# kuailehaha/liuzhou

Hardware: AMD Instinct MI355X
Metric: self-play positions/sec (fixed sims/move) (higher is better)
Workload: dtype f16

## Files before the change

include/liuzhou_hip.h:

```cpp
#ifndef LIUZHOU_HIP_H
#define LIUZHOU_HIP_H

#include <stdint.h>

#ifdef __cplusplus
extern "C" {
#endif

#if defined(_WIN32)
#define LZ_API
#else
#define LZ_API __attribute__((visibility("default")))
#endif

typedef enum LzStatus {
    LZ_OK = 0,
    LZ_ERR_ARG = -1,
    LZ_ERR_UNSUPPORTED = -2,
    LZ_ERR_LAUNCH = -3,
    LZ_ERR_ALIGN = -4,
    LZ_ERR_ILLEGAL = -5
} LzStatus;


// ... 110 lines not shown
                          float* arena_state, uint8_t* arena_legal, float* arena_policy, float* arena_value,
                          float* arena_soft, int8_t* arena_sign, void* stream);

LZ_API int lz_wave_step_finish(const LzStateSoA* states, int64_t num_slots, int64_t* plies, uint8_t* done,
                               const int32_t* chosen_action_codes, const uint8_t* terminal_mask,
                               const uint8_t* chosen_valid_mask, int64_t max_game_plies, float soft_value_k,
                               float* value_targets, float* soft_value_targets, const int8_t* player_signs,
                               const int64_t* step_index_matrix, int64_t* step_counts, int64_t max_steps,
                               int64_t* outcome, int64_t* delta_hist, int64_t* lengths, const int64_t* slot_game,
                               int64_t* finished, uint8_t* reseated, int reseat, void* stream);

LZ_API int lz_wave_reseat(const LzStateSoA* states, int64_t num_slots, uint8_t* done, int64_t* plies,
                          int64_t* step_counts, int64_t* budget, int64_t* next_game, int64_t* slot_game,
                          uint8_t* reseated, int logged_only, void* stream);

LZ_API int lz_wave_log_finished(const uint8_t* done, int64_t* step_counts, int64_t num_slots, int64_t max_steps,
                                int64_t action_dim, const float* arena_state, const uint8_t* arena_legal,
                                const float* arena_policy, const float* arena_value, const float* arena_soft,
                                float* log_state_rows, uint8_t* log_legal, float* log_policy, float* log_value,
                                float* log_soft, int64_t log_capacity, int64_t* log_state, int64_t* log_base,
                                void* stream);


#define LZ_NET_MAX_LAYERS 96
typedef struct LzNetDesc {
    int32_t channels;
    int32_t blocks;
    int32_t num_layers;
    int32_t max_blocks;
    const void* wfrag;
    const float* fparams;
    int64_t wfrag_bytes;
    int64_t fparams_bytes;
    int32_t layer_offsets[LZ_NET_MAX_LAYERS];
    int32_t head_frag_offsets[4];
    int32_t off_stem_bias, off_block0 , off_trunk_a, off_trunk_b,
            off_head_bias, off_p_gwT, off_p_a2, off_p_b2, off_p_out, off_v_w1T, off_v_b1, off_v_w2T, off_v_b2;
    int32_t flags;
    const float* wfrag_f32;
    int64_t wfrag_f32_bytes;
    const void* wfrag_lo;
    int64_t wfrag_lo_bytes;
} LzNetDesc;

LZ_API int lz_net_forward_f16(const LzNetDesc* net, const float* planes, int64_t batch,
                              float* log_p1, float* log_p2, float* log_pmc,
                              float* value_logits, float* value, void* stream);
LZ_API int lz_net_forward_packed_f16(const LzNetDesc* net, const void* packed_states, int64_t batch,
                                     float* log_p1, float* log_p2, float* log_pmc,
                                     float* value_logits, float* value, void* stream);
LZ_API int lz_net_forward_packed_counted_f16(const LzNetDesc* net, const void* packed_states, int64_t capacity,
                                             const int64_t* count, float* log_p1, float* log_p2, float* log_pmc,
                                             float* value_logits, float* value, void* stream);
LZ_API int lz_net_configure(void);
LZ_API int64_t lz_net_desc_bytes(void);
LZ_API int lz_prof_enable(int on);
LZ_API int lz_prof_net_summary(double* total_ms, int64_t* launches, int64_t* evals);
LZ_API int lz_prof_net_busy(double* busy_ms);
LZ_API int lz_prof_aux_summary(int kind, double* total_ms, int64_t* launches, int64_t* units);


typedef struct LzTreeDesc {
    int64_t num_games;
    int32_t node_cap, edge_chunk , path_cap, chunk_cap;
    double  exploration_weight;
    const void* root_state;
    void*    nodes;
    void*    edges;
    int32_t* n_nodes;
    int32_t* n_edges;
    int32_t* root_visits;
    double*  root_w;
    float*   root_init_value;
    int32_t* path;
    int32_t* path_len;
    int32_t* leaf_kind;
    void*    leaf_state;
    float*   leaf_value;
    uint8_t* root_terminal;
    const uint8_t* active;
    int32_t* leaf_edge;
    int32_t* leaf_parent;
    int32_t* trace_kind;
    void*    trace_leaf;
    float*   trace_heads;
    float*   trace_priors;
    float*   trace_value;
    int64_t  trace_cap;
    int32_t* eval_count;
    int32_t* chunk_list;
    int32_t* n_chunks;
    int32_t* free_chunks;
    int32_t* pool_top;
    int32_t* pool_stats;
    int64_t  pool_chunks;
    void*    live_state;
    int32_t* live_row;
    int64_t* live_count;
    int64_t  live_count_cap;
    int32_t* pos_index;
    float*   node_value;
    int32_t* leaf_src;
    int32_t* share_count;
    int64_t  pos_slots;
} LzTreeDesc;
LZ_API int64_t lz_tree_desc_bytes(void);
// ... 105 lines not shown
```

liuzhou_amd/csrc/lz_engine.hip:

```cpp
#include <hip/hip_runtime.h>
#include <hip/amd_detail/amd_hip_unsafe_atomics.h>
#include <math.h>
#include <stdint.h>

#include <mutex>

#include "lz_rng.h"
#include "lz_tree_dev.h"

namespace {

__global__ __launch_bounds__(kBlock) void pack_states_kernel(LzStateSoA s, int64_t B, Packed* __restrict__ out) {
    const int64_t i = (int64_t)blockIdx.x * kBlock + threadIdx.x;
    if (i >= B) return;
    State st;
    st.black = cells_equal(s.board + i * 36, 1);
    st.white = cells_equal(s.board + i * 36, -1);
    st.mb = cells_nonzero(s.marks_black + i * 36);
    st.mw = cells_nonzero(s.marks_white + i * 36);
    st.phase = (int)s.phase[i]; st.player = (int)s.current_player[i];
    st.pm_req = (int)s.pending_marks_required[i]; st.pm_rem = (int)s.pending_marks_remaining[i];
    st.pc_req = (int)s.pending_captures_required[i]; st.pc_rem = (int)s.pending_captures_remaining[i];
    st.forced = (int)s.forced_removals_done[i]; st.move_count = (int)s.move_count[i];
    st.msc = (int)s.moves_since_capture[i];
// ... 1132 lines not shown

int lz_prof_aux_begin(int kind, void* stream);
int lz_prof_aux_end(int kind, void* stream, int64_t units);

int lz_tree_advance(const LzTreeDesc* d, const int32_t* played_action, const uint8_t* reset, int64_t next_sims,
                    int32_t* dropped, int32_t* pruned, void* stream) {
    if (!tree_ok(d) || next_sims < 0) return LZ_ERR_ARG;
    if (d->num_games == 0) return LZ_OK;
    const int words = (d->node_cap + kWave - 1) / kWave;
    if (words > kMarkWordsBig) return LZ_ERR_UNSUPPORTED;
    const int64_t rn = next_sims + 1;
    if (rn > d->node_cap) return LZ_ERR_ARG;
    if ((int64_t)d->chunk_cap * (d->edge_chunk - (kMaxChildren - 1)) < (int64_t)d->node_cap * kMaxChildren) return LZ_ERR_ARG;
    const bool big = words > kMarkWordsMax;
    const int wpb = big ? 1 : kWavesPerBlock;
    const size_t lds = (size_t)wpb * (words * (sizeof(uint64_t) + sizeof(int)) + 3 * kWave * sizeof(int));
    if (big) {
        static std::mutex mu;
        static bool configured[64] = {};
        int dev = 0;
        if (hipGetDevice(&dev) != hipSuccess || dev < 0 || dev >= 64) return LZ_ERR_LAUNCH;
        std::lock_guard<std::mutex> lk(mu);
        if (!configured[dev]) {
            const size_t most = (size_t)kMarkWordsBig * (sizeof(uint64_t) + sizeof(int)) + 3 * kWave * sizeof(int);
            if (hipFuncSetAttribute(reinterpret_cast<const void*>(tree_advance_kernel<1>),
                                    hipFuncAttributeMaxDynamicSharedMemorySize, (int)most) != hipSuccess) {
                (void)hipGetLastError();
                return LZ_ERR_LAUNCH;
            }
            configured[dev] = true;
        }
    }
    (void)lz_prof_aux_begin(1, stream);
    if (big)
        hipLaunchKernelGGL(tree_advance_kernel<1>, dim3((unsigned)d->num_games), dim3(kWave), lds, as_stream(stream), make_tree(d),
                           played_action, reset, (int)rn, words, dropped, pruned, g_advance_ticks);
    else
        hipLaunchKernelGGL(tree_advance_kernel<kWavesPerBlock>, dim3(gw(d->num_games)), dim3(kBlock), lds, as_stream(stream),
                           make_tree(d), played_action, reset, (int)rn, words, dropped, pruned, g_advance_ticks);
    (void)lz_prof_aux_end(1, stream, d->num_games);
    return st();
}

static int tree_search_impl(const LzTreeDesc* d, const LzNetDesc* net, int64_t sims, float* planes, float* lp1,
                            float* lp2, float* lpmc, float* values, const float* noise, int64_t noise_stride,
                            float epsilon, bool continue_trees, void* stream) {
    if (!tree_ok(d) || !net || sims < 0 || !lp1 || !lp2 || !lpmc || !values) return LZ_ERR_ARG;
    const int64_t B = d->num_games;
    if (B == 0) return LZ_OK;
    int rc = continue_trees ? LZ_OK : lz_tree_begin(d, stream);
    if (rc) return rc;
    (void)planes;
    const Tree t = split_step(B) ? no_share(make_tree(d)) : make_tree(d);
    if (t.live_count != nullptr) {
        if (d->live_count_cap < sims + 2) return LZ_ERR_ARG;
        hipLaunchKernelGGL(tree_live_scan_kernel, dim3(1), dim3(kScanBlock), 0, as_stream(stream), t, t.live_count);
        for (int64_t s = 0; s <= sims; ++s) {
            rc = lz_net_forward_packed_counted_f16(net, d->live_state, B, d->live_count + s, lp1, lp2, lpmc, nullptr, values,
                                                   stream);
            if (rc) return rc;
            if (s == sims) {
                if (s == 0)
                    hipLaunchKernelGGL((tree_expand_kernel<true, true>), dim3(gw(t.B)), dim3(kBlock), 0, as_stream(stream), t,
                                       lp1, lp2, lpmc, (const float*)nullptr, values, noise, (int)noise_stride, epsilon, (int)s);
                else
                    hipLaunchKernelGGL((tree_expand_kernel<false, true>), dim3(gw(t.B)), dim3(kBlock), 0, as_stream(stream), t,
                                       lp1, lp2, lpmc, (const float*)nullptr, values, (const float*)nullptr, 0, 0.f, (int)s);
            } else if (s == 0) {
                hipLaunchKernelGGL((tree_expand_select_kernel<true, true>), dim3(gw(t.B)), dim3(kBlock), 0, as_stream(stream),
                                   t, lp1, lp2, lpmc, values, noise, (int)noise_stride, epsilon, (int)s);
            } else {
                (void)lz_prof_aux_begin(0, stream);
                if (split_step(t.B))
                    hipLaunchKernelGGL((tree_expand_select_split_kernel<true>), dim3(gw2(t.B)), dim3(kBlock), 0,
                                       as_stream(stream), t, lp1, lp2, lpmc, values, (int)s);
                else
                    hipLaunchKernelGGL((tree_expand_select_kernel<false, true>), dim3(gw(t.B)), dim3(kBlock), 0, as_stream(stream),
                                       t, lp1, lp2, lpmc, values, nullptr, 0, 0.f, (int)s);
                (void)lz_prof_aux_end(0, stream, B);
            }
            if (s < sims)
                hipLaunchKernelGGL(tree_live_scan_kernel, dim3(1), dim3(kScanBlock), 0, as_stream(stream), t,
                                   t.live_count + (s + 1));
        }
        return st();
    }
    for (int64_t s = 0; s <= sims; ++s) {
        rc = lz_net_forward_packed_f16(net, d->leaf_state, B, lp1, lp2, lpmc, nullptr, values, stream);
        if (rc) return rc;
        if (s == sims) {
            if (s == 0)
                hipLaunchKernelGGL(tree_expand_kernel<true>, dim3(gw(t.B)), dim3(kBlock), 0, as_stream(stream), t, lp1, lp2,
                                   lpmc, (const float*)nullptr, values, noise, (int)noise_stride, epsilon, (int)s);
            else
                hipLaunchKernelGGL(tree_expand_kernel<false>, dim3(gw(t.B)), dim3(kBlock), 0, as_stream(stream), t, lp1, lp2,
                                   lpmc, (const float*)nullptr, values, (const float*)nullptr, 0, 0.f, (int)s);
        } else if (s == 0) {
            hipLaunchKernelGGL(tree_expand_select_kernel<true>, dim3(gw(t.B)), dim3(kBlock), 0, as_stream(stream), t, lp1,
                               lp2, lpmc, values, noise, (int)noise_stride, epsilon, (int)s);
        } else {
            (void)lz_prof_aux_begin(0, stream);
            if (split_step(t.B))
                hipLaunchKernelGGL((tree_expand_select_split_kernel<false>), dim3(gw2(t.B)), dim3(kBlock), 0, as_stream(stream),
                                   t, lp1, lp2, lpmc, values, (int)s);
            else
                hipLaunchKernelGGL(tree_expand_select_kernel<false>, dim3(gw(t.B)), dim3(kBlock), 0, as_stream(stream), t, lp1,
                                   lp2, lpmc, values, nullptr, 0, 0.f, (int)s);
            (void)lz_prof_aux_end(0, stream, B);
        }
    }
    return st();
}

#ifdef LZ_EXP_TREE_STAMPS
LZ_API int lz_exp_tree_stamps(unsigned long long* out32, int reset) {
    if (out32 && hipMemcpyFromSymbol(out32, HIP_SYMBOL(g_tree_stamps), 32 * sizeof(unsigned long long)) != hipSuccess) return LZ_ERR_LAUNCH;
    if (reset) {
        unsigned long long z[32] = {};
        if (hipMemcpyToSymbol(HIP_SYMBOL(g_tree_stamps), z, sizeof(z)) != hipSuccess) return LZ_ERR_LAUNCH;
    }
    return LZ_OK;
}
#endif

int64_t lz_tree_desc_bytes(void) { return (int64_t)sizeof(LzTreeDesc); }

int lz_root_prepare(const void* root_states, int64_t B, const float* lp1, const float* lp2, const float* lpmc,
                    const float* noise, float epsilon, int64_t* legal_index_mat, float* priors_mat,
                    int32_t* action_code_mat, uint8_t* valid_mask, int32_t* counts, uint8_t* terminal_mask,
                    float* leaf_mat, void* child_states, int32_t* child_ref, uint64_t* n_children,
                    int64_t child_capacity, int32_t* overflow, void* stream) {
    if (B < 0) return LZ_ERR_ARG;
    if (B == 0) return LZ_OK;
    if (!root_states || !lp1 || !lp2 || !lpmc || !legal_index_mat || !priors_mat || !action_code_mat || !valid_mask ||
        !counts || !terminal_mask || !leaf_mat || !child_states || !child_ref || !n_children || child_capacity < 0)
        return LZ_ERR_ARG;
    if (reinterpret_cast<uintptr_t>(action_code_mat) & 15) return LZ_ERR_ALIGN;
    hipLaunchKernelGGL(zero_u64_kernel, dim3(1), dim3(64), 0, as_stream(stream),
                       reinterpret_cast<unsigned long long*>(n_children));
    hipLaunchKernelGGL(root_prepare_kernel, dim3(gw(B)), dim3(kBlock), 0, as_stream(stream),
                       reinterpret_cast<const Packed*>(root_states), B, lp1, lp2, lpmc, noise, epsilon, legal_index_mat,
// ... 122 lines not shown
```

liuzhou_amd/csrc/lz_net.hip:

```cpp
#include <hip/hip_runtime.h>
#include <algorithm>
#include <utility>
#include <vector>
#include <math.h>
#include <stdint.h>
#include <stdlib.h>

#include "../../include/liuzhou_hip.h"
#include "lz_net_dev.h"

namespace {

template <int C, int S, int W>
__global__ __launch_bounds__(W * 64, (C == 128 && W == 4) ? 1 : 2) void net_forward_kernel(NetParams P, const float* __restrict__ planes,
                                                            const uint64_t* __restrict__ packed,
                                                            int64_t N, float* __restrict__ lp1,
                                                            float* __restrict__ lp2, float* __restrict__ lpm,
                                                            float* __restrict__ vlogits, float* __restrict__ value) {
    if (P.n_dev != nullptr) { const long long nd = *P.n_dev; N = nd < N ? nd : N; }
    extern __shared__ __attribute__((aligned(16))) unsigned char lds[];
    NetCtx<C, S, W> ctx;
#ifdef LZ_EXP_HEAD_STAMPS
    ctx.t_entry = __builtin_readcyclecounter();
#endif
    net_setup<C, S, W>(P, lds, ctx);
#ifdef LZ_EXP_HEAD_STAMPS
    asm volatile("s_waitcnt vmcnt(0) lgkmcnt(0)" ::: "memory");
    ctx.t_setup = __builtin_readcyclecounter();
#endif
    const uint64_t dbg_t0 = P.debug_stop == 99 ? __builtin_readcyclecounter() : 0;
    const uint64_t dbg_w0 = P.debug_stop == 99 ? wall_clock64() : 0;
    const int64_t n_pass = (N + S - 1) / S;
    for (int64_t pass = blockIdx.x; pass < n_pass; pass += gridDim.x) {
        const int64_t n0 = pass * S;
        const int nvalid = (int)((N - n0) < S ? (N - n0) : S);
        net_pass<C, S, W>(P, lds, ctx, planes, packed, n0, nvalid, lp1, lp2, lpm, vlogits, value);
    }
    if (P.debug_stop == 99 && blockIdx.x == 7 && threadIdx.x == 0) {
        const uint64_t dt = __builtin_readcyclecounter() - dbg_t0, dw = wall_clock64() - dbg_w0;
        value[0] = (float)dt; value[1] = (float)dw;
    }
}

template <int C, int S, int W>
int launch_net(const NetParams& P, const float* planes, const uint64_t* packed, int64_t N, float* lp1, float* lp2,
               float* lpm, float* vlogits, float* value, int max_blocks, hipStream_t st) {
    using K = Cfg<C, S, W>;
    auto kern = net_forward_kernel<C, S, W>;
    const int64_t n_pass = (N + S - 1) / S;
    int grid = (int)(n_pass < max_blocks ? n_pass : max_blocks);
    if (grid < 1) grid = 1;
    hipLaunchKernelGGL(kern, dim3(grid), dim3(K::THREADS), K::LDS_BYTES, st, P, planes, packed, N, lp1, lp2, lpm, vlogits, value);
    return hipGetLastError() == hipSuccess ? LZ_OK : LZ_ERR_LAUNCH;
}

template <int C, int S, int W>
int configure_net() {
    return hipFuncSetAttribute(reinterpret_cast<const void*>(net_forward_kernel<C, S, W>),
                               hipFuncAttributeMaxDynamicSharedMemorySize, Cfg<C, S, W>::LDS_BYTES) == hipSuccess
               ? LZ_OK : LZ_ERR_LAUNCH;
}

}

namespace {
struct NetProf {
    bool on = false;
    int used = 0;
    static constexpr int kMax = 8192;
    hipEvent_t ev[2 * kMax];
    bool created = false;
    double flops = 0.0;
    int64_t evals = 0;
} g_prof;
}

extern "C" void lz_prof_aux_reset(void);

extern "C" {

int lz_prof_enable(int on) {
    if (on && !g_prof.created) {
        for (int i = 0; i < 2 * NetProf::kMax; ++i)
            if (hipEventCreate(&g_prof.ev[i]) != hipSuccess) return LZ_ERR_LAUNCH;
        g_prof.created = true;
    }
    g_prof.on = on != 0;
    g_prof.used = 0;
    g_prof.evals = 0;
    lz_prof_aux_reset();
    return LZ_OK;
}

int lz_prof_net_summary(double* total_ms, int64_t* launches, int64_t* evals) {
    double t = 0.0;
    for (int i = 0; i < g_prof.used; ++i) {
        float ms = 0.f;
        if (hipEventElapsedTime(&ms, g_prof.ev[2 * i], g_prof.ev[2 * i + 1]) != hipSuccess) return LZ_ERR_LAUNCH;
        t += ms;
    }
    if (total_ms) *total_ms = t;
    if (launches) *launches = g_prof.used;
    if (evals) *evals = g_prof.evals;
    return LZ_OK;
}

int lz_prof_net_busy(double* busy_ms) {
    if (!busy_ms) return LZ_ERR_ARG;
    *busy_ms = 0.0;
    const int n = g_prof.used;
// ... 80 lines not shown
    return a != LZ_OK ? a : (b != LZ_OK ? b : (c != LZ_OK ? c : e));
}

int lz_net_forward_f32_dispatch(const LzNetDesc* d, const float* planes, const uint64_t* packed, int64_t N, float* lp1,
                                float* lp2, float* lpmc, float* value_logits, float* value, const int64_t* n_dev,
                                void* stream);

static int net_forward_impl(const LzNetDesc* d, const float* planes, const uint64_t* packed, int64_t N, float* lp1,
                            float* lp2, float* lpmc, float* value_logits, float* value, void* stream,
                            const int64_t* n_dev = nullptr) {
    if (!d || N < 0) return LZ_ERR_ARG;
    if (N == 0) return LZ_OK;
    if (!d->wfrag || !d->fparams || (!planes && !packed)) return LZ_ERR_ARG;
    const bool heads = lp1 && lp2 && lpmc;
    if (!heads && (lp1 || lp2 || lpmc || !value)) return LZ_ERR_ARG;
    if (d->blocks < 0 || d->blocks > (LZ_NET_MAX_LAYERS - 2) / 2 || d->num_layers != 2 + 2 * d->blocks) return LZ_ERR_ARG;
    if ((reinterpret_cast<uintptr_t>(d->wfrag) & 15) || (reinterpret_cast<uintptr_t>(d->fparams) & 15)) return LZ_ERR_ALIGN;
    if (d->flags & (4 | 8))
        return lz_net_forward_f32_dispatch(d, planes, packed, N, lp1, lp2, lpmc, value_logits, value, n_dev, stream);
    NetParams P = make_net_params(d);
#ifdef LZ_EXP_SAME_LAYER
    for (int i = 3; i < 1 + 2 * d->blocks; ++i) P.layer_off[i] = d->layer_offsets[1 + ((i - 1) & 1)];
#endif
    P.n_dev = reinterpret_cast<const long long*>(n_dev);
    P.debug_stop = getenv("LZ_NET_DEBUG_STOP") ? atoi(getenv("LZ_NET_DEBUG_STOP")) : 0;
    const bool half_wg = d->channels == 64 && (d->flags & 1);
    const int max_blocks = d->max_blocks > 0 ? d->max_blocks : (half_wg ? 512 : 256);
    hipStream_t st = reinterpret_cast<hipStream_t>(stream);
    if (d->channels != 64 && d->channels != 128) return LZ_ERR_UNSUPPORTED;
    const bool prof = g_prof.on && g_prof.used < NetProf::kMax;
    if (prof) (void)hipEventRecord(g_prof.ev[2 * g_prof.used], st);
    const bool wide = d->channels == 128 && (d->flags & 2);
    const int rc = d->channels == 64
                       ? (half_wg
                              ? launch_net<64, 8, 4>(P, planes, packed, N, lp1, lp2, lpmc, value_logits, value, max_blocks, st)
                              : launch_net<64, 16, 8>(P, planes, packed, N, lp1, lp2, lpmc, value_logits, value, max_blocks, st))
                       : (wide ? launch_net<128, 8, 4>(P, planes, packed, N, lp1, lp2, lpmc, value_logits, value, max_blocks, st)
                               : launch_net<128, 8, 8>(P, planes, packed, N, lp1, lp2, lpmc, value_logits, value, max_blocks, st));
    if (prof) { (void)hipEventRecord(g_prof.ev[2 * g_prof.used + 1], st); g_prof.used += 1; g_prof.evals += N; }
    return rc;
}

int lz_net_forward_f16(const LzNetDesc* d, const float* planes, int64_t N, float* lp1, float* lp2, float* lpmc,
                       float* value_logits, float* value, void* stream) {
    return net_forward_impl(d, planes, nullptr, N, lp1, lp2, lpmc, value_logits, value, stream);
}

int lz_net_forward_packed_f16(const LzNetDesc* d, const void* packed_states, int64_t N, float* lp1, float* lp2,
                              float* lpmc, float* value_logits, float* value, void* stream) {
    return net_forward_impl(d, nullptr, reinterpret_cast<const uint64_t*>(packed_states), N, lp1, lp2, lpmc,
                            value_logits, value, stream);
}

int lz_net_forward_packed_counted_f16(const LzNetDesc* d, const void* packed_states, int64_t capacity,
                                      const int64_t* count, float* lp1, float* lp2, float* lpmc, float* value_logits,
                                      float* value, void* stream) {
    if (!count) return LZ_ERR_ARG;
    return net_forward_impl(d, nullptr, reinterpret_cast<const uint64_t*>(packed_states), capacity, lp1, lp2, lpmc,
                            value_logits, value, stream, count);
}

}
```

liuzhou_amd/csrc/lz_net_dev.h:

```cpp
#pragma once
#include <hip/hip_runtime.h>
#include <math.h>
#include <stdint.h>

#include "../../include/liuzhou_hip.h"
#include "lz_wave.h"

namespace {


typedef _Float16 h8 __attribute__((ext_vector_type(8)));
typedef _Float16 h4 __attribute__((ext_vector_type(4)));
typedef float f4 __attribute__((ext_vector_type(4)));
typedef unsigned int u4 __attribute__((ext_vector_type(4)));

struct Rsrc { __amdgpu_buffer_rsrc_t w, f; };
__device__ __forceinline__ __amdgpu_buffer_rsrc_t make_rsrc(const void* p, int bytes) {
    return __builtin_amdgcn_make_buffer_rsrc(const_cast<void*>(p), 0, bytes, 0x00020000);
}
__device__ __forceinline__ h8 load_wfrag(__amdgpu_buffer_rsrc_t r, int lane_off, int byte_off) {
    return __builtin_bit_cast(h8, __builtin_amdgcn_raw_buffer_load_b128(r, lane_off, byte_off, 0));
}
__device__ __forceinline__ f4 load_f4(__amdgpu_buffer_rsrc_t r, int lane_float_off, int float_off) {
    return __builtin_bit_cast(f4, __builtin_amdgcn_raw_buffer_load_b128(r, lane_float_off * 4, float_off * 4, 0));
// ... 364 lines not shown
__device__ __forceinline__ void fc_load(__amdgpu_buffer_rsrc_t rw, int half_off, int ct, int lane, h8 (&a)[KBN]) {
    const int wbyte = __builtin_amdgcn_readfirstlane(half_off * 2 + ct * 1024);
#pragma unroll
    for (int kb = 0; kb < KBN; ++kb) a[kb] = load_wfrag(rw, lane * 16, wbyte + kb * CTN * 1024);
}
template <int KBN>
__device__ __forceinline__ f4 fc_mma(const h8 (&a)[KBN], const unsigned char* rows, int row_stride, int lane) {
    f4 d = (f4){0.f, 0.f, 0.f, 0.f};
    const unsigned char* bp = rows + (lane & 15) * row_stride + (lane >> 4) * 16;
#pragma unroll
    for (int kb = 0; kb < KBN; ++kb)
        d = __builtin_amdgcn_mfma_f32_16x16x32_f16(a[kb], *reinterpret_cast<const h8*>(bp + kb * 64), d, 0, 0, 0);
    return d;
}
template <int CTN, int KBN>
__device__ __forceinline__ f4 fc_tile(__amdgpu_buffer_rsrc_t rw, int half_off, int ct,
                                      const unsigned char* rows, int row_stride, int lane) {
    h8 a[KBN];
    fc_load<CTN, KBN>(rw, half_off, ct, lane, a);
    return fc_mma<KBN>(a, rows, row_stride, lane);
}

template <int C, int S, int NW>
__device__ __forceinline__ void store_head(const AccT<NW>& acc, unsigned char* lds, const int (&base)[9], int map_tile0,
                                           __amdgpu_buffer_rsrc_t rf, int bias_off, int lane) {
    const int sub = (lane >> 4) * 4;
    const int delta = store_delta<C, S>(map_tile0 * 16, lane);
    f4 b[NW];
#pragma unroll
    for (int j = 0; j < NW; ++j) b[j] = load_f4(rf, sub, bias_off + (map_tile0 + j) * 16);
#pragma unroll
    for (int i = 0; i < 9; ++i) {
#pragma unroll
        for (int j = 0; j < NW; ++j) {
            const f4 v = acc[i][j] + b[j];
            *reinterpret_cast<h4*>(lds + base[i] + delta + store_off(j)) = relu_h4(v);
        }
    }
}

template <int C, int S, int W>
struct NetCtx {
    int tid, lane, wave, pg, cg, ct0, chan0;
    __amdgpu_buffer_rsrc_t rw, rf;
    int base[9];
    bool mirror;
    int row_step;
#ifdef LZ_EXP_HEAD_STAMPS
    uint64_t t_entry, t_setup;
#endif
};

template <int C, int S, int W>
__device__ __forceinline__ void net_setup(const NetParams& P, unsigned char* lds, NetCtx<C, S, W>& ctx) {
    using K = Cfg<C, S, W>;
    static_assert(K::CT == K::CG * K::CTW && (K::CTW == 2 || K::CTW == 4), "each wave owns 2 or 4 output-channel tiles");
    static_assert(K::NT % 9 == 0 && K::PG * K::CG == K::WAVES, "waves = cell groups x channel groups");
    static_assert(S * 32 <= K::THREADS, "global pooling uses 2 lanes per (sample, 4-channel group)");
    constexpr int NTHR = K::THREADS;
    const int tid = threadIdx.x;
    const int lane = tid & 63;
    const int wave = __builtin_amdgcn_readfirstlane(tid >> 6);
    const int pg = wave % K::PG, cg = wave / K::PG;
    const int tile0 = pg * 9;
    ctx.tid = tid; ctx.lane = lane; ctx.wave = wave; ctx.pg = pg; ctx.cg = cg;
    ctx.ct0 = cg * K::CTW;
    ctx.chan0 = ctx.ct0 * 16;
    ctx.rw = make_rsrc(P.wfrag, P.wfrag_bytes);
    ctx.rf = make_rsrc(P.fp, P.fparams_bytes);
#pragma unroll
    for (int i = 0; i < 9; ++i) {
        const int n = tile_cell_calc(pg, i, lane & 15);
        ctx.base[i] = K::ACT_OFF + board_row(n) * K::STRIDE + (lane >> 4) * 32 - K::STRIDE;
    }
    ctx.mirror = (pg & 1) != 0;
    ctx.row_step = ctx.mirror ? -7 * K::STRIDE : 7 * K::STRIDE;
    for (int i = tid; i < K::ZERO_OFF / 16; i += NTHR) reinterpret_cast<uint4*>(lds + K::ACT_OFF)[i] = make_uint4(0, 0, 0, 0);
    for (int i = tid; i < (K::PAR_OFF - K::POOL_OFF) / 4; i += NTHR) reinterpret_cast<uint32_t*>(lds + K::POOL_OFF)[i] = 0u;
}

template <int C, int S, int W>
__device__ __forceinline__ void net_pass(const NetParams& P, unsigned char* lds, NetCtx<C, S, W>& ctx, const float* planes,
                                         const uint64_t* packed, int64_t n0, int nvalid, float* lp1, float* lp2,
                                         float* lpm, float* vlogits, float* value) {
    using K = Cfg<C, S, W>;
    constexpr int NW = K::CTW;
    using Acc = AccT<NW>;
    constexpr int NTHR = K::THREADS;
    const int tid = ctx.tid, lane = ctx.lane, wave = ctx.wave, cg = ctx.cg, ct0 = ctx.ct0, chan0 = ctx.chan0;
    const float* fp = P.fp;
    const __amdgpu_buffer_rsrc_t rw = ctx.rw, rf = ctx.rf;
    int (&base)[9] = ctx.base;
    const bool mirror = ctx.mirror;
    const int row_step = ctx.row_step;
    float* gvec = reinterpret_cast<float*>(lds + K::G_OFF);
    float* plog = reinterpret_cast<float*>(lds + K::PLOG_OFF);
    float* par = reinterpret_cast<float*>(lds + K::PAR_OFF);
    int tid_s = tid;
    asm volatile("" : "+v"(tid_s));
    const int st_s = tid_s >> 5, st_p = tid_s & 31;
    uint64_t rec0 = 0, rec1 = 0, rec2 = 0, rec3 = 0;
    if (packed != nullptr && st_s < nvalid) {
        const uint64_t* rec = packed + (n0 + st_s) * 4;
        rec0 = rec[0]; rec1 = rec[1]; rec2 = rec[2]; rec3 = rec[3];
    }
#ifdef LZ_EXP_HEAD_STAMPS
    asm volatile("s_waitcnt vmcnt(0) lgkmcnt(0)" ::: "memory");
    const uint64_t t_before_barrier = __builtin_readcyclecounter();
#endif
    __syncthreads();
#ifdef LZ_EXP_HEAD_STAMPS
    const uint64_t t_after_barrier = __builtin_readcyclecounter();
    uint64_t fst[4] = {0, 0, 0, 0};
#define LZ_FSTAMP(k) { asm volatile("s_waitcnt vmcnt(0) lgkmcnt(0)" ::: "memory"); fst[k] = __builtin_readcyclecounter(); }
#else
#define LZ_FSTAMP(k)
#endif
    LZ_FSTAMP(0)
    if (packed != nullptr) {
        if (st_s < S) {
            const bool on = st_s < nvalid;
            const bool white = (rec0 >> 53) & 1;
            const int phase = on ? (int)((rec0 >> 50) & 7) : 0;
            const uint64_t own = white ? rec1 : rec0, opp = white ? rec0 : rec1;
            const uint64_t sm = white ? rec3 : rec2, om = white ? rec2 : rec3;
            for (int p = st_p; p < 36; p += 32) {
                _Float16 row[32];
#pragma unroll
                for (int k = 0; k < 32; ++k) row[k] = (_Float16)0.f;
                if (on) {
                    row[0] = (_Float16)(float)((own >> p) & 1);
                    row[1] = (_Float16)(float)((opp >> p) & 1);
                    row[2] = (_Float16)(float)((sm >> p) & 1);
                    row[3] = (_Float16)(float)((om >> p) & 1);
#pragma unroll
                    for (int ph = 1; ph <= 7; ++ph) row[3 + ph] = (_Float16)(phase == ph ? 1.f : 0.f);
                }
                const int n = st_s * 36 + p;
#pragma unroll
                for (int q = 0; q < 4; ++q) {
                    h8 v;
#pragma unroll
                    for (int k = 0; k < 8; ++k) v[k] = row[q * 8 + k];
                    *reinterpret_cast<h8*>(lds + act_addr<C, S>(n, q)) = v;
                }
            }
        }
    } else {
        for (int n = tid_s; n < K::NPOS; n += NTHR) {
            const int s = n / 36, p = n - s * 36;
            _Float16 row[32];
#pragma unroll
            for (int k = 0; k < 32; ++k) row[k] = (_Float16)0.f;
            if (s < nvalid) {
                const float* src = planes + (n0 + s) * 396 + p;
#pragma unroll
                for (int ch = 0; ch < 11; ++ch) row[ch] = (_Float16)src[ch * 36];
            }
#pragma unroll
            for (int q = 0; q < 4; ++q) {
                h8 v;
#pragma unroll
                for (int k = 0; k < 8; ++k) v[k] = row[q * 8 + k];
                *reinterpret_cast<h8*>(lds + act_addr<C, S>(n, q)) = v;
            }
        }
    }
    LZ_FSTAMP(1)
    __syncthreads();
    LZ_FSTAMP(2)
    if (P.debug_stop == 1) return;

    Acc x, acc;
#pragma unroll
    for (int i = 0; i < 9; ++i)
#pragma unroll
        for (int j = 0; j < NW; ++j) x[i][j] = (f4){0.f, 0.f, 0.f, 0.f};
    h8 Af[NW];
    f4 pa[NW], pb[NW];
    load_first_frags<C, S, true, true, K::CT, NW>(rw, P.layer_off[0], ct0, lane, Af);
    load_chan_params<NW>(rf, P.stem_bias, chan0, lane, pb);
    conv_gemm<C, S, true, true, K::CT, NW>(x, rw, P.layer_off[0], ct0, lds, base, lane, Af, mirror, row_step);
#pragma unroll
    for (int j = 0; j < NW; ++j) {
#pragma unroll
        for (int i = 0; i < 9; ++i) {
            f4 v = x[i][j] + pb[j];
            x[i][j] = (f4){fmaxf(v[0], 0.f), fmaxf(v[1], 0.f), fmaxf(v[2], 0.f), fmaxf(v[3], 0.f)};
        }
    }
    LZ_FSTAMP(3)
    if (P.debug_stop == 2) { if (lane == 0 && x[0][0][0] == 123.f) lp1[0] = 1.f; return; }
#ifdef LZ_EXP_HEAD_STAMPS
#define LZ_HSTAMP(k) { asm volatile("s_waitcnt vmcnt(0) lgkmcnt(0)" ::: "memory"); hstamps[k] = __builtin_readcyclecounter(); }
    uint64_t hstamps[16] = {0, 0, 0, 0, 0, 0, 0, 0, 0, 0, 0, 0, 0, 0, 0, 0};
#else
#define LZ_HSTAMP(k)
#endif
#ifdef LZ_EXP_STAMPS
#define LZ_STAMP(k) if (blk == 2) { asm volatile("s_waitcnt lgkmcnt(0)" ::: "memory"); stamps[k] = __builtin_readcyclecounter(); }
    uint64_t stamps[9] = {0, 0, 0, 0, 0, 0, 0, 0, 0};
#else
#define LZ_STAMP(k)
#endif
    for (int blk = 0; blk < P.blocks; ++blk) {
        const int bp = P.blk0 + blk * 3 * C;
        load_chan_params<NW>(rf, bp, chan0, lane, pa);
        load_chan_params<NW>(rf, bp + C, chan0, lane, pb);
// ... 88 lines not shown
#pragma unroll
            for (int hf = 0; hf < 2; ++hf) {
                const int ch = (kb * 4 + (lane_h >> 4)) * 8 + hf * 4;
                pa2[kb][hf] = *reinterpret_cast<const f4*>(par + ch);
                pb2[kb][hf] = *reinterpret_cast<const f4*>(par + kHead + ch);
            }
        for (int t = wave; t < K::NT; t += K::WAVES) {
            f4 d = (f4){0.f, 0.f, 0.f, 0.f};
            const int n = t * 16 + (lane_h & 15);
            const int s = n / 36, p = n - s * 36;
#pragma unroll
            for (int kb = 0; kb < 2; ++kb) {
                const int chunk = kb * 4 + (lane_h >> 4);
                const h8 v = *reinterpret_cast<const h8*>(lds + act_addr<C, S>(n, chunk));
                const f4 g0 = *reinterpret_cast<const f4*>(gvec + s * kHead + chunk * 8);
                const f4 g1 = *reinterpret_cast<const f4*>(gvec + s * kHead + chunk * 8 + 4);
                const h4 lo = __builtin_shufflevector(v, v, 0, 1, 2, 3), hi = __builtin_shufflevector(v, v, 4, 5, 6, 7);
                const h4 r0 = relu_h4((__builtin_convertvector(lo, f4) + g0) * pa2[kb][0] + pb2[kb][0]);
                const h4 r1 = relu_h4((__builtin_convertvector(hi, f4) + g1) * pa2[kb][1] + pb2[kb][1]);
                const h8 b = __builtin_shufflevector(r0, r1, 0, 1, 2, 3, 4, 5, 6, 7);
                d = __builtin_amdgcn_mfma_f32_16x16x32_f16(kb == 0 ? wo0 : wo1, b, d, 0, 0, 0);
            }
            if (lane_h < 16) {
                plog[(s * 3 + 0) * 36 + p] = d[0];
                plog[(s * 3 + 1) * 36 + p] = d[1];
                plog[(s * 3 + 2) * 36 + p] = d[2];
            }
        }
    }
    __syncthreads();
    LZ_HSTAMP(5)
    {
        constexpr int ROWS = S * 3, PASSES = (ROWS + 4 * K::WAVES - 1) / (4 * K::WAVES);
        const int k4 = lane_h & 15;
#pragma unroll
        for (int pass = 0; pass < PASSES; ++pass) {
            const int row = (pass * K::WAVES + wave) * 4 + (lane_h >> 4);
            const bool on = k4 < 9 && row < ROWS;
            const f4 v = on ? *reinterpret_cast<const f4*>(plog + row * 36 + 4 * k4) : (f4){-INFINITY, -INFINITY, -INFINITY, -INFINITY};
            float mx = fmaxf(fmaxf(v[0], v[1]), fmaxf(v[2], v[3]));
            mx = fmaxf(mx, lzw::dpp_f32<0x128, 0xf>(mx, mx));
            mx = fmaxf(mx, lzw::dpp_f32<0x124, 0xf>(mx, mx));
            mx = fmaxf(mx, lzw::dpp_f32<0x122, 0xf>(mx, mx));
            mx = fmaxf(mx, lzw::dpp_f32<0x121, 0xf>(mx, mx));
            float e = 0.f;
            if (on) e = ((expf(v[0] - mx) + expf(v[1] - mx)) + expf(v[2] - mx)) + expf(v[3] - mx);
            e += lzw::dpp_f32<0x128, 0xf>(e, e);
            e += lzw::dpp_f32<0x124, 0xf>(e, e);
            e += lzw::dpp_f32<0x122, 0xf>(e, e);
            e += lzw::dpp_f32<0x121, 0xf>(e, e);
            const int s = row / 3, h = row - s * 3;
            if (on && s < nvalid) {
                const float lse = mx + logf(e);
                float* dst = (h == 0 ? lp1 : h == 1 ? lp2 : lpm) + (n0 + s) * 36 + 4 * k4;
                dst[0] = v[0] - lse; dst[1] = v[1] - lse; dst[2] = v[2] - lse; dst[3] = v[3] - lse;
            }
        }
    }
    __syncthreads();
    LZ_HSTAMP(6)
    }
    if (P.debug_stop == 5) { if (lane_h == 0 && x[0][0][0] == 123.f) lp1[0] = 1.f; return; }
    if (K::HP == 2) store_head<C, S, NW>(x, lds, base, ht1 - 4, rf, P.head_bias + kHead, lane);
    else if (ht0 >= 4) store_head<C, S, NW>(acc, lds, base, ht0 - 4, rf, P.head_bias + kHead, lane);
    constexpr int R1 = (8 + K::WAVES - 1) / K::WAVES, R2 = (7 + K::WAVES - 1) / K::WAVES;
    h8 w1[R1][6], w2[R2][4];
    f4 b1[R1], b2[R2];
#pragma unroll
    for (int r = 0; r < R1; ++r) {
        const int ct = wave + r * K::WAVES < 8 ? wave + r * K::WAVES : 7;
        fc_load<8, 6>(rw, P.hf_w1, ct, lane_h, w1[r]);
        b1[r] = load_f4(rf, (lane_h >> 4) * 4, P.v_b1 + ct * 16);
    }
#pragma unroll
    for (int r = 0; r < R2; ++r) {
        const int ct = wave + r * K::WAVES < 7 ? wave + r * K::WAVES : 6;
        fc_load<7, 4>(rw, P.hf_w2, ct, lane_h, w2[r]);
        b2[r] = load_f4(rf, (lane_h >> 4) * 4, P.v_b2 + ct * 16);
    }
    __syncthreads();
    LZ_HSTAMP(7)
    gpool64<C, S>(lds, tid_h);
    __syncthreads();
    LZ_HSTAMP(8)
#pragma unroll
    for (int r = 0; r < R1; ++r) {
        const int ct = wave + r * K::WAVES;
        if (ct < 8) {
            const f4 v = fc_mma<6>(w1[r], lds + K::POOL_OFF, K::POOL_STRIDE, lane_h) + b1[r];
            const int s = lane_h & 15, ch = ct * 16 + (lane_h >> 4) * 4;
            *reinterpret_cast<h4*>(lds + K::HID_OFF + s * K::HID_STRIDE + ch * 2) =
                to_h4(fmaxf(v[0], 0.f), fmaxf(v[1], 0.f), fmaxf(v[2], 0.f), fmaxf(v[3], 0.f));
        }
    }
    __syncthreads();
    LZ_HSTAMP(9)
    float* vl = plog;
#pragma unroll
    for (int r = 0; r < R2; ++r) {
        const int ct = wave + r * K::WAVES;
        if (ct < 7) {
            const f4 d = fc_mma<4>(w2[r], lds + K::HID_OFF, K::HID_STRIDE, lane_h);
            const int s = lane_h & 15, o = ct * 16 + (lane_h >> 4) * 4;
#pragma unroll
            for (int q = 0; q < 4; ++q)
                if (o + q < kBins) vl[s * K::VL_STRIDE + o + q] = d[q] + b2[r][q];
        }
    }
    __syncthreads();
    LZ_HSTAMP(10)
    {
        constexpr int SPW = (S + K::WAVES - 1) / K::WAVES;
        float v0[SPW], v1[SPW], mx[SPW], e0[SPW], e1[SPW], sum[SPW], ex[SPW];
#pragma unroll
        for (int i = 0; i < SPW; ++i) {
            const int s = wave + i * K::WAVES;
            const bool on = s < nvalid;
            v0[i] = on ? vl[s * K::VL_STRIDE + lane_h] : 0.f;
            v1[i] = (on && lane_h + 64 < kBins) ? vl[s * K::VL_STRIDE + lane_h + 64] : -INFINITY;
        }
#pragma unroll
        for (int i = 0; i < SPW; ++i) mx[i] = lzw::wave_max(fmaxf(v0[i], v1[i]));
#pragma unroll
        for (int i = 0; i < SPW; ++i) {
            e0[i] = expf(v0[i] - mx[i]);
            e1[i] = lane_h + 64 < kBins ? expf(v1[i] - mx[i]) : 0.f;
        }
#pragma unroll
        for (int i = 0; i < SPW; ++i) sum[i] = lzw::wave_sum(e0[i] + e1[i]);
#pragma unroll
        for (int i = 0; i < SPW; ++i)
            ex[i] = lzw::wave_sum(e0[i] * (-1.0f + 0.02f * (float)lane_h) + e1[i] * (-1.0f + 0.02f * (float)(lane_h + 64)));
#pragma unroll
        for (int i = 0; i < SPW; ++i) {
            const int s = wave + i * K::WAVES;
            if (s < nvalid) {
                if (lane_h == 0 && value != nullptr) value[n0 + s] = ex[i] / sum[i];
                if (vlogits != nullptr) {
                    vlogits[(n0 + s) * kBins + lane_h] = v0[i];
                    if (lane_h + 64 < kBins) vlogits[(n0 + s) * kBins + lane_h + 64] = v1[i];
                }
            }
        }
    }
#ifdef LZ_EXP_HEAD_STAMPS
    LZ_HSTAMP(11)
    __syncthreads();
    if (blockIdx.x == 0 && lane_h == 0 && vlogits != nullptr) {
        for (int k = 0; k < 12; ++k) vlogits[wave * 24 + k] = (float)(hstamps[k] - hstamps[0]);
        vlogits[wave * 24 + 12] = (float)(ctx.t_setup - ctx.t_entry);
        vlogits[wave * 24 + 13] = (float)(fst[0] - ctx.t_setup);
        vlogits[wave * 24 + 14] = (float)(fst[1] - fst[0]);
        vlogits[wave * 24 + 15] = (float)(fst[2] - fst[1]);
        vlogits[wave * 24 + 16] = (float)(fst[3] - fst[2]);
        vlogits[wave * 24 + 17] = (float)(hstamps[0] - fst[3]);
        vlogits[wave * 24 + 18] = (float)(t_before_barrier - ctx.t_setup);
        vlogits[wave * 24 + 19] = (float)(t_after_barrier - t_before_barrier);
        vlogits[wave * 24 + 20] = (float)(ctx.t_entry & 0xFFFFFF);
    }
#endif
}

inline NetParams make_net_params(const LzNetDesc* d) {
    NetParams P;
    P.wfrag = reinterpret_cast<const _Float16*>(d->wfrag);
    P.fp = d->fparams;
    for (int i = 0; i < LZ_NET_MAX_LAYERS; ++i) P.layer_off[i] = i < d->num_layers ? d->layer_offsets[i] : 0;
    P.blocks = d->blocks;
    P.n_dev = nullptr;
    P.wfrag_bytes = (int)d->wfrag_bytes; P.fparams_bytes = (int)d->fparams_bytes;
    P.debug_stop = 0;
    P.hf_gw = d->head_frag_offsets[0]; P.hf_w1 = d->head_frag_offsets[1]; P.hf_w2 = d->head_frag_offsets[2];
    P.hf_out = d->head_frag_offsets[3];
    P.stem_bias = d->off_stem_bias; P.blk0 = d->off_block0; P.trunk_a = d->off_trunk_a; P.trunk_b = d->off_trunk_b;
    P.head_bias = d->off_head_bias; P.p_gwT = d->off_p_gwT; P.p_a2 = d->off_p_a2; P.p_b2 = d->off_p_b2;
    P.p_out = d->off_p_out; P.v_w1T = d->off_v_w1T; P.v_b1 = d->off_v_b1; P.v_w2T = d->off_v_w2T; P.v_b2 = d->off_v_b2;
    return P;
}

}
```

Baseline: 12760.

## Fuse live-leaf compaction into net forward via flagged gather kernel

Adds a flagged net-forward kernel that reads per-game leaf kinds, builds a ballot bitmask and prefix sums in LDS, and evaluates only live leaves by gathering their rows. The tree search uses it in place of the separate live-scan kernel plus counted forward when the net flags allow. This removes a serial single-block scan launch per simulation and skips evaluating non-live leaves. In exchange every block redundantly scans the whole kind array and runs a binary search per row, and the gather leaves memory access scattered.

Result: no change. 12880, median of 6 (+1.0%).

```diff
diff --git a/include/liuzhou_hip.h b/include/liuzhou_hip.h
--- a/include/liuzhou_hip.h
+++ b/include/liuzhou_hip.h
@@ -186,6 +186,9 @@
 LZ_API int lz_net_forward_packed_counted_f16(const LzNetDesc* net, const void* packed_states, int64_t capacity,
                                              const int64_t* count, float* log_p1, float* log_p2, float* log_pmc,
                                              float* value_logits, float* value, void* stream);
+LZ_API int lz_net_forward_packed_flagged_f16(const LzNetDesc* net, const void* packed_states, const int32_t* kinds,
+                                             int64_t batch, int64_t* count, float* log_p1, float* log_p2,
+                                             float* log_pmc, float* value_logits, float* value, void* stream);
 LZ_API int lz_net_configure(void);
 LZ_API int64_t lz_net_desc_bytes(void);
 LZ_API int lz_prof_enable(int on);
diff --git a/liuzhou_amd/csrc/lz_engine.hip b/liuzhou_amd/csrc/lz_engine.hip
--- a/liuzhou_amd/csrc/lz_engine.hip
+++ b/liuzhou_amd/csrc/lz_engine.hip
@@ -1208,8 +1208,9 @@
     if (rc) return rc;
     (void)planes;
     const Tree t = split_step(B) ? no_share(make_tree(d)) : make_tree(d);
-    if (t.live_count != nullptr) {
-        if (d->live_count_cap < sims + 2) return LZ_ERR_ARG;
+    const bool flagged = t.live_count != nullptr && !(net->flags & (4 | 8));
+    if (t.live_count != nullptr && d->live_count_cap < sims + 2) return LZ_ERR_ARG;
+    if (t.live_count != nullptr && !flagged) {
         hipLaunchKernelGGL(tree_live_scan_kernel, dim3(1), dim3(kScanBlock), 0, as_stream(stream), t, t.live_count);
         for (int64_t s = 0; s <= sims; ++s) {
             rc = lz_net_forward_packed_counted_f16(net, d->live_state, B, d->live_count + s, lp1, lp2, lpmc, nullptr, values,
@@ -1242,7 +1243,9 @@
         return st();
     }
     for (int64_t s = 0; s <= sims; ++s) {
-        rc = lz_net_forward_packed_f16(net, d->leaf_state, B, lp1, lp2, lpmc, nullptr, values, stream);
+        rc = flagged ? lz_net_forward_packed_flagged_f16(net, d->leaf_state, t.leaf_kind, B, d->live_count + s, lp1, lp2,
+                                                         lpmc, nullptr, values, stream)
+                     : lz_net_forward_packed_f16(net, d->leaf_state, B, lp1, lp2, lpmc, nullptr, values, stream);
         if (rc) return rc;
         if (s == sims) {
             if (s == 0)
diff --git a/liuzhou_amd/csrc/lz_net.hip b/liuzhou_amd/csrc/lz_net.hip
--- a/liuzhou_amd/csrc/lz_net.hip
+++ b/liuzhou_amd/csrc/lz_net.hip
@@ -54,8 +54,123 @@
     return hipGetLastError() == hipSuccess ? LZ_OK : LZ_ERR_LAUNCH;
 }
 
+constexpr int kFlagLive = 1;
+constexpr int kFlagRows = 256;
+constexpr int kFlagUnroll = 32;
+
+template <int C, int S, int W>
+struct FlagCfg {
+    static constexpr int ROWS_OFF = (Cfg<C, S, W>::LDS_BYTES + 15) & ~15;
+    static constexpr int LDS_BYTES = ROWS_OFF + kFlagRows * 4;
+    static constexpr int MAX_PASSES = kFlagRows / S;
+    static constexpr int scratch_bytes(int nwords) { return (nwords * 12 + W * 4 + 15) & ~15; }
+};
+
+template <int C, int S, int W>
+__global__ __launch_bounds__(W * 64, (C == 128 && W == 4) ? 1 : 2) void net_forward_flagged_kernel(
+    NetParams P, const uint64_t* __restrict__ packed, const int* __restrict__ kind, int B,
+    unsigned long long* __restrict__ count_out, float* __restrict__ lp1, float* __restrict__ lp2, float* __restrict__ lpm,
+    float* __restrict__ vlogits, float* __restrict__ value) {
+    using K = Cfg<C, S, W>;
+    using F = FlagCfg<C, S, W>;
+    constexpr int NTHR = K::THREADS;
+    static_assert(NTHR >= kFlagRows, "one thread per row of the workgroup's game list");
+    extern __shared__ __attribute__((aligned(16))) unsigned char lds[];
+    const int tid = threadIdx.x, lane = tid & 63;
+    const int wave = __builtin_amdgcn_readfirstlane(tid >> 6);
+    const int nwords = (B + 63) >> 6;
+    uint64_t* mask = reinterpret_cast<uint64_t*>(lds + K::ACT_OFF);
+    int* pre = reinterpret_cast<int*>(lds + K::ACT_OFF + nwords * 8);
+    int* wsum = pre + nwords;
+    int* rows = reinterpret_cast<int*>(lds + F::ROWS_OFF);
+    const int scratch = F::scratch_bytes(nwords);
+    const __amdgpu_buffer_rsrc_t kr = make_rsrc(kind, B * 4);
+    int kv[kFlagUnroll];
+    auto load = [&](int i0) {
+#pragma unroll
+        for (int u = 0; u < kFlagUnroll; ++u)
+            kv[u] = (int)__builtin_amdgcn_raw_buffer_load_b32(kr, ((i0 + u * W) * 64 + lane) * 4, 0, 0);
+    };
+    auto flag = [&](int i0) {
+#pragma unroll
+        for (int u = 0; u < kFlagUnroll; ++u) {
+            const int i = i0 + u * W;
+            const uint64_t m = __ballot(kv[u] == kFlagLive);
+            if (i < nwords && lane == 0) mask[i] = m;
+        }
+    };
+    load(wave);
+    NetCtx<C, S, W> ctx;
+    net_setup<C, S, W>(P, lds, ctx, scratch);
+    flag(wave);
+    for (int i0 = wave + kFlagUnroll * W; i0 < nwords; i0 += kFlagUnroll * W) { load(i0); flag(i0); }
+    __syncthreads();
+    const int q = (nwords + NTHR - 1) / NTHR, w0 = tid * q, w1 = w0 + q < nwords ? w0 + q : nwords;
+    int cnt = 0;
+    for (int i = w0; i < w1; ++i) cnt += __popcll(mask[i]);
+    int incl = cnt;
+#pragma unroll
+    for (int d = 1; d < 64; d <<= 1) {
+        const int v = __shfl_up(incl, d, 64);
+        if (lane >= d) incl += v;
+    }
+    if (lane == 63) wsum[wave] = incl;
+    __syncthreads();
+    int run = incl - cnt, total = 0;
+    for (int i = 0; i < W; ++i) { run += i < wave ? wsum[i] : 0; total += wsum[i]; }
+    for (int i = w0; i < w1; ++i) { pre[i] = run; run += __popcll(mask[i]); }
+    __syncthreads();
+    const int n_pass = (total + S - 1) / S;
+    if (tid < kFlagRows) {
+        const int k = tid / S, p = blockIdx.x + k * gridDim.x, r = p * S + (tid - k * S);
+        if (p < n_pass && r < total) {
+            int lo = 0, hi = nwords - 1;
+            while (lo < hi) {
+                const int mid = (lo + hi + 1) >> 1;
+                if (pre[mid] <= r) lo = mid; else hi = mid - 1;
+            }
+            uint64_t m = mask[lo];
+            int n = r - pre[lo], pos = 0;
+#pragma unroll
+            for (int half = 32; half >= 1; half >>= 1) {
+                const uint64_t low = m & ((1ull << half) - 1);
+                const int c = __popcll(low);
+                if (n >= c) { n -= c; m >>= half; pos += half; } else m = low;
+            }
+            rows[tid] = lo * 64 + pos;
+        }
+    }
+    if (blockIdx.x == 0 && tid == 0) *count_out = (unsigned long long)total;
+    __syncthreads();
+    for (int i = tid; i < scratch / 16; i += NTHR) reinterpret_cast<uint4*>(lds + K::ACT_OFF)[i] = make_uint4(0, 0, 0, 0);
+    for (int p = blockIdx.x, k = 0; p < n_pass; p += gridDim.x, ++k) {
+        const int nvalid = total - p * S < S ? total - p * S : S;
+        net_pass<C, S, W, true>(P, lds, ctx, nullptr, packed, 0, nvalid, lp1, lp2, lpm, vlogits, value, rows + k * S);
+    }
+}
+
+template <int C, int S, int W>
+int launch_net_flagged(const NetParams& P, const uint64_t* packed, const int* kind, int B, unsigned long long* count,
+                       float* lp1, float* lp2, float* lpm, float* vlogits, float* value, int max_blocks, hipStream_t st) {
+    using K = Cfg<C, S, W>;
+    using F = FlagCfg<C, S, W>;
+    const int64_t nwords = ((int64_t)B + 63) / 64;
+    if (F::scratch_bytes((int)nwords) > K::ZERO_OFF - K::ACT_OFF) return LZ_ERR_UNSUPPORTED;
+    const int64_t n_pass = ((int64_t)B + S - 1) / S;
+    int64_t grid = n_pass < max_blocks ? n_pass : max_blocks;
+    const int64_t need = (n_pass + F::MAX_PASSES - 1) / F::MAX_PASSES;
+    if (grid < need) grid = need;
+    if (grid < 1) grid = 1;
+    hipLaunchKernelGGL((net_forward_flagged_kernel<C, S, W>), dim3((unsigned)grid), dim3(K::THREADS), F::LDS_BYTES, st, P,
+                       packed, kind, B, count, lp1, lp2, lpm, vlogits, value);
+    return hipGetLastError() == hipSuccess ? LZ_OK : LZ_ERR_LAUNCH;
+}
+
 template <int C, int S, int W>
 int configure_net() {
+    if (hipFuncSetAttribute(reinterpret_cast<const void*>(net_forward_flagged_kernel<C, S, W>),
+                            hipFuncAttributeMaxDynamicSharedMemorySize, FlagCfg<C, S, W>::LDS_BYTES) != hipSuccess)
+        return LZ_ERR_LAUNCH;
     return hipFuncSetAttribute(reinterpret_cast<const void*>(net_forward_kernel<C, S, W>),
                                hipFuncAttributeMaxDynamicSharedMemorySize, Cfg<C, S, W>::LDS_BYTES) == hipSuccess
                ? LZ_OK : LZ_ERR_LAUNCH;
@@ -242,6 +357,36 @@
                             value_logits, value, stream);
 }
 
+int lz_net_forward_packed_flagged_f16(const LzNetDesc* d, const void* packed_states, const int32_t* kinds, int64_t B,
+                                      int64_t* count, float* lp1, float* lp2, float* lpmc, float* value_logits,
+                                      float* value, void* stream) {
+    if (!d || !packed_states || !kinds || !count || B < 0 || B > INT32_MAX) return LZ_ERR_ARG;
+    hipStream_t st = reinterpret_cast<hipStream_t>(stream);
+    if (B == 0) return hipMemsetAsync(count, 0, sizeof(int64_t), st) == hipSuccess ? LZ_OK : LZ_ERR_LAUNCH;
+    if (!d->wfrag || !d->fparams) return LZ_ERR_ARG;
+    const bool heads = lp1 && lp2 && lpmc;
+    if (!heads && (lp1 || lp2 || lpmc || !value)) return LZ_ERR_ARG;
+    if (d->blocks < 0 || d->blocks > (LZ_NET_MAX_LAYERS - 2) / 2 || d->num_layers != 2 + 2 * d->blocks) return LZ_ERR_ARG;
+    if ((reinterpret_cast<uintptr_t>(d->wfrag) & 15) || (reinterpret_cast<uintptr_t>(d->fparams) & 15)) return LZ_ERR_ALIGN;
+    if (d->flags & (4 | 8)) return LZ_ERR_UNSUPPORTED;
+    if (d->channels != 64 && d->channels != 128) return LZ_ERR_UNSUPPORTED;
+    NetParams P = make_net_params(d);
+    const bool half_wg = d->channels == 64 && (d->flags & 1), wide = d->channels == 128 && (d->flags & 2);
+    const int max_blocks = d->max_blocks > 0 ? d->max_blocks : (half_wg ? 512 : 256);
+    const uint64_t* packed = reinterpret_cast<const uint64_t*>(packed_states);
+    unsigned long long* cnt = reinterpret_cast<unsigned long long*>(count);
+    const int b = (int)B;
+    const bool prof = g_prof.on && g_prof.used < NetProf::kMax;
+    if (prof) (void)hipEventRecord(g_prof.ev[2 * g_prof.used], st);
+    const int rc = d->channels == 64
+                       ? (half_wg ? launch_net_flagged<64, 8, 4>(P, packed, kinds, b, cnt, lp1, lp2, lpmc, value_logits, value, max_blocks, st)
+                                  : launch_net_flagged<64, 16, 8>(P, packed, kinds, b, cnt, lp1, lp2, lpmc, value_logits, value, max_blocks, st))
+                       : (wide ? launch_net_flagged<128, 8, 4>(P, packed, kinds, b, cnt, lp1, lp2, lpmc, value_logits, value, max_blocks, st)
+                               : launch_net_flagged<128, 8, 8>(P, packed, kinds, b, cnt, lp1, lp2, lpmc, value_logits, value, max_blocks, st));
+    if (prof) { (void)hipEventRecord(g_prof.ev[2 * g_prof.used + 1], st); g_prof.used += 1; g_prof.evals += B; }
+    return rc;
+}
+
 int lz_net_forward_packed_counted_f16(const LzNetDesc* d, const void* packed_states, int64_t capacity,
                                       const int64_t* count, float* lp1, float* lp2, float* lpmc, float* value_logits,
                                       float* value, void* stream) {
diff --git a/liuzhou_amd/csrc/lz_net_dev.h b/liuzhou_amd/csrc/lz_net_dev.h
--- a/liuzhou_amd/csrc/lz_net_dev.h
+++ b/liuzhou_amd/csrc/lz_net_dev.h
@@ -440,7 +440,7 @@
 };
 
 template <int C, int S, int W>
-__device__ __forceinline__ void net_setup(const NetParams& P, unsigned char* lds, NetCtx<C, S, W>& ctx) {
+__device__ __forceinline__ void net_setup(const NetParams& P, unsigned char* lds, NetCtx<C, S, W>& ctx, int zero_from = 0) {
     using K = Cfg<C, S, W>;
     static_assert(K::CT == K::CG * K::CTW && (K::CTW == 2 || K::CTW == 4), "each wave owns 2 or 4 output-channel tiles");
     static_assert(K::NT % 9 == 0 && K::PG * K::CG == K::WAVES, "waves = cell groups x channel groups");
@@ -463,14 +463,15 @@
     }
     ctx.mirror = (pg & 1) != 0;
     ctx.row_step = ctx.mirror ? -7 * K::STRIDE : 7 * K::STRIDE;
-    for (int i = tid; i < K::ZERO_OFF / 16; i += NTHR) reinterpret_cast<uint4*>(lds + K::ACT_OFF)[i] = make_uint4(0, 0, 0, 0);
+    for (int i = zero_from / 16 + tid; i < K::ZERO_OFF / 16; i += NTHR)
+        reinterpret_cast<uint4*>(lds + K::ACT_OFF)[i] = make_uint4(0, 0, 0, 0);
     for (int i = tid; i < (K::PAR_OFF - K::POOL_OFF) / 4; i += NTHR) reinterpret_cast<uint32_t*>(lds + K::POOL_OFF)[i] = 0u;
 }
 
-template <int C, int S, int W>
+template <int C, int S, int W, bool GATHER = false>
 __device__ __forceinline__ void net_pass(const NetParams& P, unsigned char* lds, NetCtx<C, S, W>& ctx, const float* planes,
                                          const uint64_t* packed, int64_t n0, int nvalid, float* lp1, float* lp2,
-                                         float* lpm, float* vlogits, float* value) {
+                                         float* lpm, float* vlogits, float* value, const int* rows = nullptr) {
     using K = Cfg<C, S, W>;
     constexpr int NW = K::CTW;
     using Acc = AccT<NW>;
@@ -481,6 +482,7 @@
     int (&base)[9] = ctx.base;
     const bool mirror = ctx.mirror;
     const int row_step = ctx.row_step;
+    auto row_of = [&](int s) -> int64_t { return GATHER ? (int64_t)rows[s] : n0 + s; };
     float* gvec = reinterpret_cast<float*>(lds + K::G_OFF);
     float* plog = reinterpret_cast<float*>(lds + K::PLOG_OFF);
     float* par = reinterpret_cast<float*>(lds + K::PAR_OFF);
@@ -489,7 +491,7 @@
     const int st_s = tid_s >> 5, st_p = tid_s & 31;
     uint64_t rec0 = 0, rec1 = 0, rec2 = 0, rec3 = 0;
     if (packed != nullptr && st_s < nvalid) {
-        const uint64_t* rec = packed + (n0 + st_s) * 4;
+        const uint64_t* rec = packed + row_of(st_s) * 4;
         rec0 = rec[0]; rec1 = rec[1]; rec2 = rec[2]; rec3 = rec[3];
     }
 #ifdef LZ_EXP_HEAD_STAMPS
@@ -541,7 +543,7 @@
 #pragma unroll
             for (int k = 0; k < 32; ++k) row[k] = (_Float16)0.f;
             if (s < nvalid) {
-                const float* src = planes + (n0 + s) * 396 + p;
+                const float* src = planes + row_of(s) * 396 + p;
 #pragma unroll
                 for (int ch = 0; ch < 11; ++ch) row[ch] = (_Float16)src[ch * 36];
             }
@@ -736,7 +738,7 @@
             const int s = row / 3, h = row - s * 3;
             if (on && s < nvalid) {
                 const float lse = mx + logf(e);
-                float* dst = (h == 0 ? lp1 : h == 1 ? lp2 : lpm) + (n0 + s) * 36 + 4 * k4;
+                float* dst = (h == 0 ? lp1 : h == 1 ? lp2 : lpm) + row_of(s) * 36 + 4 * k4;
                 dst[0] = v[0] - lse; dst[1] = v[1] - lse; dst[2] = v[2] - lse; dst[3] = v[3] - lse;
             }
         }
@@ -819,10 +821,11 @@
         for (int i = 0; i < SPW; ++i) {
             const int s = wave + i * K::WAVES;
             if (s < nvalid) {
-                if (lane_h == 0 && value != nullptr) value[n0 + s] = ex[i] / sum[i];
+                const int64_t r = row_of(s);
+                if (lane_h == 0 && value != nullptr) value[r] = ex[i] / sum[i];
                 if (vlogits != nullptr) {
-                    vlogits[(n0 + s) * kBins + lane_h] = v0[i];
-                    if (lane_h + 64 < kBins) vlogits[(n0 + s) * kBins + lane_h + 64] = v1[i];
+                    vlogits[r * kBins + lane_h] = v0[i];
+                    if (lane_h + 64 < kBins) vlogits[r * kBins + lane_h + 64] = v1[i];
                 }
             }
         }
```
